# distributed-information-bottleneck/distributed-information-bottleneck.github.io

Hardware: NVIDIA H100
Metric: training samples/sec (16-feat synthetic, batch 65k) at 1/2/4/8 H100; HBM GB/s (higher is better)
Workload: dtype fp16 operands + fp32 accumulate (wgmma f16; PE/exp/KL/loss/Adam fp32)

## Files before the change

### distributed-information-bottleneck.github.io_b200/csrc/dib_enc_fused.cu

```cuda
#include <cuda.h>
#include <cuda_bf16.h>
#include <cuda_fp16.h>

#include "dib_common.cuh"
#include "dib_kernels.h"
#include "dib_sm90.cuh"

namespace {

using namespace sm90;

constexpr int TM = 128;
constexpr int HID = 128;
constexpr int EO = 64;
constexpr int K0 = 16;
constexpr int kThreads = 256;
constexpr int kPanel = TM * 128;

constexpr int kW0Elems = K0 * HID, kW1Elems = HID * HID, kW2Elems = HID * EO, kB1Elems = K0 * HID, kB2Elems = K0 * EO;
constexpr int kPackElems = kW0Elems + kW1Elems + kW2Elems + kB1Elems + kB2Elems;

constexpr int kOffW1 = 0;
constexpr int kOffW2 = kOffW1 + 2 * kPanel;
constexpr int kOffW0 = kOffW2 + kPanel;
constexpr int kOffBb1 = kOffW0 + 2 * K0 * 128;
constexpr int kOffBb2 = kOffBb1 + 2 * K0 * 128;
constexpr int kA0Bytes = 2 * TM * 16;
constexpr int kOffA0 = kOffBb2 + K0 * 128;
constexpr int kOffX = kOffA0 + 2 * kA0Bytes;
constexpr int kOffFwdEnd = kOffX + kThreads * 16;
constexpr int kOffH1 = kOffFwdEnd;
constexpr int kOffH2 = kOffH1 + 2 * kPanel;
constexpr int kOffDO = kOffH2 + 2 * kPanel;
constexpr int kOffDZ2 = kOffDO + kPanel;
constexpr int kOffG = kOffDZ2 + 2 * kPanel;
constexpr int kOffBwdEnd = kOffG + TM * 64;
static_assert(kOffH1 % 1024 == 0 && kOffDZ2 % 1024 == 0, "operand tiles must be 1024-byte aligned");

struct EncFusedParams {
  const float* x; int ldx;
  const int* x_off;
  const int* fdim;
  int nfreq;
  const float* params;
  const long long* b1_off; const long long* b2_off;
  const float* eps;
  unsigned long long seed; unsigned int step; unsigned long long sample_offset;
  const unsigned int* step_dev;
  float* emb; int ldemb; float* user_emb;
  uint16_t* emb16; int ldemb16;
  float* kl_part; int kl_stride;
  int F; long long n; int act; float alpha;
  int round_emb;
};

template <bool BF16>
__device__ __forceinline__ uint32_t pack2(float a, float b) {
  uint32_t r;
  if constexpr (BF16) asm("cvt.rn.satfinite.bf16x2.f32 %0, %1, %2;" : "=r"(r) : "f"(b), "f"(a));
  else asm("cvt.rn.satfinite.f16x2.f32 %0, %1, %2;" : "=r"(r) : "f"(b), "f"(a));
  return r;
}

template <bool BF16>
__device__ __forceinline__ uint32_t pack2_relu(float a, float b) {
  uint32_t r;
  if constexpr (BF16) asm("cvt.rn.relu.satfinite.bf16x2.f32 %0, %1, %2;" : "=r"(r) : "f"(b), "f"(a));
  else asm("cvt.rn.relu.satfinite.f16x2.f32 %0, %1, %2;" : "=r"(r) : "f"(b), "f"(a));
  return r;
}

template <bool BF16>
__device__ __forceinline__ void unpack2(uint32_t u, float& a, float& b) {
  if constexpr (BF16) { const float2 f = __bfloat1622float2(*reinterpret_cast<__nv_bfloat162*>(&u)); a = f.x; b = f.y; }
  else { const float2 f = __half22float2(*reinterpret_cast<__half2*>(&u)); a = f.x; b = f.y; }
}

__device__ __forceinline__ void st_shared_v4(uint32_t addr, uint32_t a, uint32_t b, uint32_t c, uint32_t d) {
  asm volatile("st.shared.v4.b32 [%0], {%1, %2, %3, %4};" ::"r"(addr), "r"(a), "r"(b), "r"(c), "r"(d) : "memory");
}
__device__ __forceinline__ void st_shared_b32(uint32_t addr, uint32_t v) {
  asm volatile("st.shared.b32 [%0], %1;" ::"r"(addr), "r"(v) : "memory");
}
__device__ __forceinline__ uint32_t ld_shared_b32(uint32_t addr) {
  uint32_t v;
  asm volatile("ld.shared.b32 %0, [%1];" : "=r"(v) : "r"(addr) : "memory");
  return v;
}

__device__ __forceinline__ uint32_t tile_chunk_addr(uint32_t tile, int r, int col) {
  const int panel = col >> 6, c = (col & 63) >> 3;
  return tile + panel * kPanel + r * 128 + ((c ^ (r & 7)) << 4);
}

struct Frag {
  int rb, q;
};
__device__ __forceinline__ Frag frag_of(int tid) {
  const int wg = tid >> 7, wq = (tid >> 5) & 3, lane = tid & 31;
  return Frag{64 * wg + 16 * wq + (lane >> 2), lane & 3};
}

template <bool BF16, bool RELU, int N>
__device__ __forceinline__ void frag_to_tile(const float (&d)[N / 2], uint32_t tile, Frag fr, int act, float alpha) {
#pragma unroll
  for (int j = 0; j < N / 8; ++j) {
#pragma unroll
    for (int h = 0; h < 2; ++h) {
      const float v0 = d[4 * j + 2 * h], v1 = d[4 * j + 2 * h + 1];
      const uint32_t w = RELU ? pack2_relu<BF16>(v0, v1) : pack2<BF16>(dib_act16(act, v0, alpha), dib_act16(act, v1, alpha));
      st_shared_b32(tile_chunk_addr(tile, fr.rb + 8 * h, 8 * j) + 4 * fr.q, w);
    }
  }
}

template <bool BF16, bool RELU, int N>
__device__ __forceinline__ void frag_to_a(const float (&d)[N / 2], uint32_t (&a)[N / 4], int act, float alpha) {
#pragma unroll
  for (int j = 0; j < N / 8; ++j) {
#pragma unroll
    for (int h = 0; h < 2; ++h) {
      const float v0 = d[4 * j + 2 * h], v1 = d[4 * j + 2 * h + 1];
      a[2 * j + h] = RELU ? pack2_relu<BF16>(v0, v1) : pack2<BF16>(dib_act16(act, v0, alpha), dib_act16(act, v1, alpha));
    }
  }
}

template <bool BF16>
__device__ __forceinline__ uint32_t relu_gate2(uint32_t p, uint32_t h) {
  if constexpr (BF16) {
    const __nv_bfloat162 z = __float2bfloat162_rn(0.f);
    __nv_bfloat162 g = __hmul2(*reinterpret_cast<__nv_bfloat162*>(&p), __hgt2(*reinterpret_cast<__nv_bfloat162*>(&h), z));
    return *reinterpret_cast<uint32_t*>(&g);
  } else {
    const __half2 z = __float2half2_rn(0.f);
    __half2 g = __hmul2(*reinterpret_cast<__half2*>(&p), __hgt2(*reinterpret_cast<__half2*>(&h), z));
    return *reinterpret_cast<uint32_t*>(&g);
  }
}

template <bool BF16, bool RELU>
__device__ __forceinline__ void frag_dgrad_to_tile(const float (&d)[64], uint32_t htile, uint32_t dtile, Frag fr, int act,
                                                   float alpha) {
#pragma unroll
  for (int j = 0; j < 16; ++j) {
#pragma unroll
    for (int h = 0; h < 2; ++h) {
      const uint32_t off = tile_chunk_addr(0u, fr.rb + 8 * h, 8 * j) + 4 * fr.q;
      const uint32_t hv = ld_shared_b32(htile + off);
      const float g0 = d[4 * j + 2 * h], g1 = d[4 * j + 2 * h + 1];
      uint32_t o;
      if constexpr (RELU) {
        o = relu_gate2<BF16>(pack2<BF16>(g0, g1), hv);
      } else {
        float h0, h1;
        unpack2<BF16>(hv, h0, h1);
        o = pack2<BF16>(g0 * dib_act_grad(act, h0, alpha), g1 * dib_act_grad(act, h1, alpha));
      }
      st_shared_b32(dtile + off, o);
    }
  }
}

__device__ __forceinline__ float dib_sin_pe(float a) {
  float t = a * 0.15915494309189535f;
  t -= rintf(t);
  return __sinf(6.283185307179586f * t);
}
constexpr int kMaxFeatDim = 3;
template <bool BF16>
__device__ __forceinline__ void write_a0_row(uint32_t a0, int r, int khalf, bool valid, const float (&xv)[kMaxFeatDim], int d,
                                             int nfreq) {
  float f[8];
  const int w_in = d * nfreq;
  int blk = (khalf * 8) / d, j = khalf * 8 - blk * d;
#pragma unroll
  for (int k = 0; k < 8; ++k) {
    const int col = khalf * 8 + k;
    float v = 0.f;
    if (col < w_in) {
      float xj = xv[0];
#pragma unroll
      for (int q = 1; q < kMaxFeatDim; ++q) if (j == q) xj = xv[q];
      v = blk == 0 ? xj : dib_sin_pe((float)(1 << blk) * xj);
    } else if (col == w_in) {
      v = valid ? 1.f : 0.f;
    }
    f[k] = v;
    if (++j == d) { j = 0; ++blk; }
  }
  st_shared_v4(a0 + khalf * (TM * 16) + r * 16, pack2<BF16>(f[0], f[1]), pack2<BF16>(f[2], f[3]), pack2<BF16>(f[4], f[5]),
               pack2<BF16>(f[6], f[7]));
}

__device__ __forceinline__ int a0_row(int tid) { return 64 * (tid >> 7) + (tid & 63); }

__device__ __forceinline__ void prefetch_x(const EncFusedParams& P, uint32_t xs, int tid, long long row0, int d, int xo) {
  const long long grow = row0 + a0_row(tid);
  if (grow < P.n) {
    const float* src = P.x + grow * P.ldx + xo;
#pragma unroll
    for (int j = 0; j < kMaxFeatDim; ++j)
      if (j < d) cp_async_4(xs + 4 * j, src + j);
  }
  cp_async_commit();
}
template <bool BF16>
__device__ __forceinline__ void stage_a0(const EncFusedParams& P, uint32_t a0, const float* xslot, int tid, long long row0,
                                         int d) {
  const int ar = a0_row(tid), khalf = (tid >> 6) & 1;
  const long long grow = row0 + ar;
  cp_async_wait_all();
  float xv[kMaxFeatDim];
#pragma unroll
  for (int j = 0; j < kMaxFeatDim; ++j) xv[j] = (grow < P.n && j < d) ? xslot[j] : 0.f;
  write_a0_row<BF16>(a0, ar, khalf, grow < P.n, xv, d, P.nfreq);
}

__device__ __forceinline__ void noise_pair(const EncFusedParams& P, unsigned int step, long long grow_lo, int f, int j, int q,
                                           int lane, float (&nz)[2][2]) {
  if (P.eps) {
#pragma unroll
    for (int h = 0; h < 2; ++h) {
      const long long grow = grow_lo + 8 * h;
      if (grow < P.n) {
        const float2 e = *reinterpret_cast<const float2*>(P.eps + (grow * P.F + f) * 32 + 8 * j + 2 * q);
        nz[h][0] = e.x; nz[h][1] = e.y;
      } else {
        nz[h][0] = nz[h][1] = 0.f;
      }
    }
    return;
  }
  float n4[4];
  dib_philox_normal4(P.seed, step, P.sample_offset + (unsigned long long)(grow_lo + 8 * (q & 1)), (uint32_t)f,
                     (uint32_t)(2 * j + (q >> 1)), n4);
#pragma unroll
  for (int h = 0; h < 2; ++h) {
    const int src = (lane & ~3) | ((q >> 1) << 1) | h;
    float t[4];
#pragma unroll
    for (int k = 0; k < 4; ++k) t[k] = __shfl_sync(0xffffffffu, n4[k], src);
    nz[h][0] = (q & 1) ? t[2] : t[0];
    nz[h][1] = (q & 1) ? t[3] : t[1];
  }
}

struct WeightMaps { CUtensorMap w0, w1, w2, b1, b2; };

__device__ __forceinline__ void load_weights(uint32_t sb, const WeightMaps& m, uint32_t bar, int f) {
  mbar_expect_tx(bar, 2 * K0 * 128 + 2 * kPanel + kPanel + 2 * K0 * 128 + K0 * 128);
  tma_load_3d(sb + kOffW0, &m.w0, bar, 0, 0, f);
  tma_load_3d(sb + kOffW0 + K0 * 128, &m.w0, bar, 64, 0, f);
  tma_load_3d(sb + kOffW1, &m.w1, bar, 0, 0, f);
  tma_load_3d(sb + kOffW1 + kPanel, &m.w1, bar, 64, 0, f);
  tma_load_3d(sb + kOffW2, &m.w2, bar, 0, 0, f);
  tma_load_3d(sb + kOffBb1, &m.b1, bar, 0, 0, f);
  tma_load_3d(sb + kOffBb1 + K0 * 128, &m.b1, bar, 64, 0, f);
  tma_load_3d(sb + kOffBb2, &m.b2, bar, 0, 0, f);
}

__device__ __forceinline__ uint64_t desc_a0_as_a(uint32_t a0, int wg) { return gmma_desc(a0 + wg * 64 * 16, TM * 16, 128, kLayoutNone); }
__device__ __forceinline__ uint64_t desc_a0_as_b(uint32_t a0, int kk) { return gmma_desc(a0 + kk * 256, 128, TM * 16, kLayoutNone); }
__device__ __forceinline__ uint64_t desc_act_as_a(uint32_t tile, int wg, int kk) {
  return gmma_desc(tile + (kk >> 2) * kPanel + wg * 64 * 128 + (kk & 3) * 32, 16, 1024);
}
__device__ __forceinline__ uint64_t desc_act_t_as_a(uint32_t tile, int p, int kk) { return gmma_desc(tile + p * kPanel + kk * 2048, kPanel, 1024); }
__device__ __forceinline__ uint64_t desc_act_as_b(uint32_t tile, int kk) { return gmma_desc(tile + kk * 2048, kPanel, 1024); }

template <bool BF16>
__device__ __forceinline__ void mma_layer0(float (&d)[64], uint32_t sb, uint32_t a0, int wg) {
  wgmma_m64n128k16<BF16, 0, 1>(d, desc_a0_as_a(a0, wg), gmma_desc(sb + kOffW0, K0 * 128, 1024), 0u);
}
template <bool BF16>
__device__ __forceinline__ void mma_layer1(float (&d)[64], uint32_t sb, uint32_t h1, uint32_t a0, int wg) {
  wgmma_m64n128k16<BF16, 0, 1>(d, desc_a0_as_a(a0, wg), gmma_desc(sb + kOffBb1, K0 * 128, 1024), 0u);
#pragma unroll
  for (int kk = 0; kk < HID / 16; ++kk)
    wgmma_m64n128k16<BF16, 0, 1>(d, desc_act_as_a(h1, wg, kk), gmma_desc(sb + kOffW1 + kk * 2048, kPanel, 1024), 1u);
}
template <bool BF16>
__device__ __forceinline__ void mma_layer2(float (&d)[32], uint32_t sb, uint32_t h2, uint32_t a0, int wg) {
  wgmma_m64n64k16<BF16, 0, 1>(d, desc_a0_as_a(a0, wg), gmma_desc(sb + kOffBb2, K0 * 128, 1024), 0u);
#pragma unroll
  for (int kk = 0; kk < HID / 16; ++kk)
    wgmma_m64n64k16<BF16, 0, 1>(d, desc_act_as_a(h2, wg, kk), gmma_desc(sb + kOffW2 + kk * 2048, kPanel, 1024), 1u);
}
template <bool BF16>
__device__ __forceinline__ void mma_layer1_rs(float (&d)[64], uint32_t sb, const uint32_t (&h1)[32], uint32_t a0, int wg) {
  wgmma_m64n128k16<BF16, 0, 1>(d, desc_a0_as_a(a0, wg), gmma_desc(sb + kOffBb1, K0 * 128, 1024), 0u);
#pragma unroll
  for (int kk = 0; kk < HID / 16; ++kk) {
    const uint32_t a[4] = {h1[4 * kk], h1[4 * kk + 1], h1[4 * kk + 2], h1[4 * kk + 3]};
    wgmma_m64n128k16_rs<BF16, 1>(d, a, gmma_desc(sb + kOffW1 + kk * 2048, kPanel, 1024), 1u);
  }
}
template <bool BF16>
__device__ __forceinline__ void mma_layer2_rs(float (&d)[32], uint32_t sb, const uint32_t (&h2)[32], uint32_t a0, int wg) {
  wgmma_m64n64k16<BF16, 0, 1>(d, desc_a0_as_a(a0, wg), gmma_desc(sb + kOffBb2, K0 * 128, 1024), 0u);
#pragma unroll
  for (int kk = 0; kk < HID / 16; ++kk) {
    const uint32_t a[4] = {h2[4 * kk], h2[4 * kk + 1], h2[4 * kk + 2], h2[4 * kk + 3]};
    wgmma_m64n64k16_rs<BF16, 1>(d, a, gmma_desc(sb + kOffW2 + kk * 2048, kPanel, 1024), 1u);
  }
}

__device__ __forceinline__ void wg_publish(int wg) {
  fence_proxy_async_smem();
  named_bar_sync(1 + wg, 128);
}
__device__ __forceinline__ void cta_publish() {
  fence_proxy_async_smem();
  __syncthreads();
}

struct Sched { int f_first, f_step, slot, nslots; };
__device__ __forceinline__ Sched sched_of(int c, int G, int F) {
  if (G >= F) { const int f0 = c % F; return Sched{f0, F * G, c / F, (G - f0 + F - 1) / F}; }
  return Sched{c, G, 0, 1};
}

template <bool BF16, bool RELU>
__global__ void __launch_bounds__(kThreads, 2)
dib_enc_fused_fwd_kernel(const __grid_constant__ WeightMaps maps, const EncFusedParams P) {
  extern __shared__ uint8_t smem_raw[];
  const uint32_t sb = (smem_u32(smem_raw) + 1023u) & ~1023u;
  uint8_t* sg = smem_raw + (sb - smem_u32(smem_raw));
  float* red_s = reinterpret_cast<float*>(sg + kOffFwdEnd + 64);
  const uint32_t bar_w = sb + kOffFwdEnd;

  const int tid = threadIdx.x, warp = tid >> 5, lane = tid & 31, wg = tid >> 7;
  const Frag fr = frag_of(tid);
  const int F = P.F;
  const int ntiles = (int)((P.n + TM - 1) / TM);
  const unsigned int nstep = P.step + (P.step_dev ? P.step_dev[0] : 0u);
  const uint32_t a0 = sb + kOffA0, xs = sb + kOffX + tid * 16;
  const float* xslot = reinterpret_cast<const float*>(sg + kOffX + tid * 16);

  if (tid == 0) {
    tma_prefetch_desc(&maps.w0); tma_prefetch_desc(&maps.w1); tma_prefetch_desc(&maps.w2);
    tma_prefetch_desc(&maps.b1); tma_prefetch_desc(&maps.b2);
    mbar_init(bar_w, 1);
    fence_barrier_init();
  }
  __syncthreads();

  const Sched s = sched_of(blockIdx.x, gridDim.x, F);
  uint32_t fit = 0;
  for (int f = s.f_first; f < F; f += s.f_step, ++fit) {
    if (tid == 0) load_weights(sb, maps, bar_w, f);
    const int d = P.fdim[f], xo = P.x_off[f];
    prefetch_x(P, xs, tid, (long long)s.slot * TM, d, xo);
    float kl_acc = 0.f;
    mbar_wait(bar_w, fit & 1);
    for (int t = s.slot; t < ntiles; t += s.nslots) {
      const long long row0 = (long long)t * TM;
      stage_a0<BF16>(P, a0, xslot, tid, row0, d);
      prefetch_x(P, xs, tid, row0 + (long long)s.nslots * TM, d, xo);
      wg_publish(wg);
      float acc[64];
      uint32_t ha[32];
      wgmma_fence();
      mma_layer0<BF16>(acc, sb, a0, wg);
      wgmma_commit();
      wgmma_wait<0>();
      wgmma_fence_regs(acc);
      frag_to_a<BF16, RELU, 128>(acc, ha, P.act, P.alpha);
      wgmma_fence();
      mma_layer1_rs<BF16>(acc, sb, ha, a0, wg);
      wgmma_commit();
      wgmma_wait<0>();
      wgmma_fence_regs(acc);
      frag_to_a<BF16, RELU, 128>(acc, ha, P.act, P.alpha);
      float acc2[32];
      wgmma_fence();
      mma_layer2_rs<BF16>(acc2, sb, ha, a0, wg);
      wgmma_commit();
      const long long grow_lo = row0 + fr.rb;
      float nz[4][2][2];
#pragma unroll
      for (int j = 0; j < 4; ++j) noise_pair(P, nstep, grow_lo, f, j, fr.q, lane, nz[j]);
      wgmma_wait<0>();
      wgmma_fence_regs(acc2);
#pragma unroll
      for (int h = 0; h < 2; ++h) {
        const long long grow = grow_lo + 8 * h;
        if (grow >= P.n) continue;
#pragma unroll
        for (int j = 0; j < 4; ++j) {
          const int e = 8 * j + 2 * fr.q;
          float u[2];
#pragma unroll
          for (int k = 0; k < 2; ++k) {
            const float mu = acc2[4 * j + 2 * h + k], lv = acc2[4 * (j + 4) + 2 * h + k];
            const float sv = __expf(0.5f * lv);
            u[k] = fmaf(sv, nz[j][h][k], mu);
            kl_acc += 0.5f * (mu * mu + sv * sv - lv - 1.f);
          }
          if (P.user_emb) *reinterpret_cast<float2*>(P.user_emb + grow * ((long long)F * 32) + f * 32 + e) = make_float2(u[0], u[1]);
          if (P.emb16) *reinterpret_cast<uint32_t*>(P.emb16 + grow * P.ldemb16 + f * 32 + e) = pack2<BF16>(u[0], u[1]);
          if (P.emb) {
            const float2 o = P.round_emb ? make_float2(dib_round_tf32(u[0]), dib_round_tf32(u[1])) : make_float2(u[0], u[1]);
            *reinterpret_cast<float2*>(P.emb + grow * P.ldemb + f * 32 + e) = o;
          }
        }
      }
    }
    kl_acc = dib_warp_sum(kl_acc);
    if (lane == 0) red_s[warp] = kl_acc;
    __syncthreads();
    if (tid == 0) {
      float sum = 0.f;
      for (int i = 0; i < kThreads / 32; ++i) sum += red_s[i];
      P.kl_part[(long long)f * P.kl_stride + s.slot] = sum;
    }
    __syncthreads();
  }
}

struct EncFusedBwdParams {
  EncFusedParams f;
  const float* d_emb; int ldd;
  const uint16_t* d_emb16;
  const float* beta_dev; float inv_batch; float gscale;
  float* part; long long split_stride;
  const long long* w0_off; const long long* b0_off; const long long* w1_off; const long long* w2_off;
};

__device__ __forceinline__ void load_demb16(uint32_t dst, const CUtensorMap* gmap, uint32_t bar, int f, long long row0) {
  mbar_expect_tx(bar, TM * 64);
  tma_load_2d(dst, gmap, bar, f * 32, (int)row0);
}

template <bool BF16, bool RELU>
__global__ void __launch_bounds__(kThreads, 1)
dib_enc_fused_bwd_kernel(const __grid_constant__ WeightMaps maps, const __grid_constant__ CUtensorMap gmap,
                         const EncFusedBwdParams Q) {
  const EncFusedParams& P = Q.f;
  extern __shared__ uint8_t smem_raw[];
  const uint32_t sb = (smem_u32(smem_raw) + 1023u) & ~1023u;
  const uint8_t* sg = smem_raw + (sb - smem_u32(smem_raw));
  const uint32_t bar_w = sb + kOffBwdEnd, bar_g = bar_w + 8;

  const int tid = threadIdx.x, lane = tid & 31, wg = tid >> 7;
  const Frag fr = frag_of(tid);
  const int F = P.F;
  const int ntiles = (int)((P.n + TM - 1) / TM);
  const unsigned int nstep = P.step + (P.step_dev ? P.step_dev[0] : 0u);
  const uint32_t h1 = sb + kOffH1, h2 = sb + kOffH2, dO = sb + kOffDO, dz2 = sb + kOffDZ2, gbuf = sb + kOffG;
  const uint32_t xs = sb + kOffX + tid * 16;
  const float* xslot = reinterpret_cast<const float*>(sg + kOffX + tid * 16);
  const uint32_t* gsm = reinterpret_cast<const uint32_t*>(sg + kOffG);
  const float S = Q.gscale, invS = 1.f / Q.gscale;

  if (tid == 0) {
    tma_prefetch_desc(&maps.w0); tma_prefetch_desc(&maps.w1); tma_prefetch_desc(&maps.w2);
    tma_prefetch_desc(&maps.b1); tma_prefetch_desc(&maps.b2);
    if (Q.d_emb16) tma_prefetch_desc(&gmap);
    mbar_init(bar_w, 1);
    mbar_init(bar_g, 1);
    fence_barrier_init();
  }
  __syncthreads();

  const Sched s = sched_of(blockIdx.x, gridDim.x, F);
  uint32_t fit = 0, tpar = 0;
  for (int f = s.f_first; f < F; f += s.f_step, ++fit) {
    if (tid == 0) {
      load_weights(sb, maps, bar_w, f);
      if (Q.d_emb16 && s.slot < ntiles) load_demb16(gbuf, &gmap, bar_g, f, (long long)s.slot * TM);
    }
    const int d = P.fdim[f], xo = P.x_off[f];
    prefetch_x(P, xs, tid, (long long)s.slot * TM, d, xo);
    const float bs = Q.beta_dev[0] * Q.inv_batch * S;
    float accW1[64], accW2[32], accW0[8], accB1[8], accB2[8];
    mbar_wait(bar_w, fit & 1);
    for (int t = s.slot; t < ntiles; t += s.nslots) {
      const long long row0 = (long long)t * TM;
      const uint32_t wacc = t != s.slot;
      const uint32_t a0 = sb + kOffA0 + tpar * kA0Bytes;
      stage_a0<BF16>(P, a0, xslot, tid, row0, d);
      prefetch_x(P, xs, tid, row0 + (long long)s.nslots * TM, d, xo);
      wg_publish(wg);
      float acc[64];
      wgmma_fence();
      mma_layer0<BF16>(acc, sb, a0, wg);
      wgmma_commit();
      wgmma_wait<0>();
      wgmma_fence_regs(acc); wgmma_fence_regs(accW0);
      frag_to_tile<BF16, RELU, 128>(acc, h1, fr, P.act, P.alpha);
      cta_publish();
      wgmma_fence();
      mma_layer1<BF16>(acc, sb, h1, a0, wg);
      wgmma_commit();
      wgmma_wait<0>();
      wgmma_fence_regs(acc);
      frag_to_tile<BF16, RELU, 128>(acc, h2, fr, P.act, P.alpha);
      wg_publish(wg);
      float acc2[32];
      wgmma_fence();
      mma_layer2<BF16>(acc2, sb, h2, a0, wg);
      wgmma_commit();
      const long long grow_lo = row0 + fr.rb;
      float nz[4][2][2];
#pragma unroll
      for (int j = 0; j < 4; ++j) noise_pair(P, nstep, grow_lo, f, j, fr.q, lane, nz[j]);
      if (Q.d_emb16) mbar_wait(bar_g, tpar);
      wgmma_wait<0>();
      wgmma_fence_regs(acc2);
#pragma unroll
      for (int h = 0; h < 2; ++h) {
        const long long grow = grow_lo + 8 * h;
        const bool valid = grow < P.n;
        const float bsv = valid ? bs : 0.f;
        const int r = fr.rb + 8 * h;
#pragma unroll
        for (int j = 0; j < 4; ++j) {
          const int e = 8 * j + 2 * fr.q;
          float g[2] = {0.f, 0.f};
          if (valid) {
            if (Q.d_emb16) unpack2<BF16>(gsm[r * 16 + e / 2], g[0], g[1]);
            else {
              const float2 g2 = *reinterpret_cast<const float2*>(Q.d_emb + grow * Q.ldd + f * 32 + e);
              g[0] = g2.x * S; g[1] = g2.y * S;
            }
          }
          float dm[2], dl[2];
#pragma unroll
          for (int k = 0; k < 2; ++k) {
            const float mu = acc2[4 * j + 2 * h + k], lv = acc2[4 * (j + 4) + 2 * h + k];
            const float sgm = expf(0.5f * lv);
            dm[k] = fmaf(bsv, mu, g[k]);
            dl[k] = valid ? fmaf(g[k] * nz[j][h][k], 0.5f * sgm, bsv * 0.5f * (sgm * sgm - 1.f)) : 0.f;
          }
          st_shared_b32(tile_chunk_addr(dO, r, e) + 4 * fr.q, pack2<BF16>(dm[0], dm[1]));
          st_shared_b32(tile_chunk_addr(dO, r, 32 + e) + 4 * fr.q, pack2<BF16>(dl[0], dl[1]));
        }
      }
      cta_publish();
      if (tid == 0 && Q.d_emb16 && t + s.nslots < ntiles) load_demb16(gbuf, &gmap, bar_g, f, row0 + (long long)s.nslots * TM);
      wgmma_fence();
#pragma unroll
      for (int kk = 0; kk < EO / 16; ++kk)
        wgmma_m64n128k16<BF16, 0, 0>(acc, gmma_desc(dO + wg * 64 * 128 + kk * 32, 16, 1024),
                                     gmma_desc(sb + kOffW2 + kk * 32, 16, 1024), kk > 0 ? 1u : 0u);
      wgmma_commit();
#pragma unroll
      for (int kk = 0; kk < TM / 16; ++kk)
        wgmma_m64n64k16<BF16, 1, 1>(accW2, desc_act_t_as_a(h2, wg, kk), desc_act_as_b(dO, kk), kk > 0 ? 1u : wacc);
#pragma unroll
      for (int kk = 0; kk < TM / 16; ++kk)
        wgmma_m64n16k16<BF16, 1, 1>(accB2, desc_act_t_as_a(dO, 0, kk), desc_a0_as_b(a0, kk), kk > 0 ? 1u : wacc);
      wgmma_commit();
      wgmma_wait<1>();
      wgmma_fence_regs(acc);
      frag_dgrad_to_tile<BF16, RELU>(acc, h2, dz2, fr, P.act, P.alpha);
      wgmma_wait<0>();
      wgmma_fence_regs(accW2); wgmma_fence_regs(accB2);
      cta_publish();
      wgmma_fence();
#pragma unroll
      for (int kk = 0; kk < HID / 16; ++kk)
        wgmma_m64n128k16<BF16, 0, 0>(acc, desc_act_as_a(dz2, wg, kk),
                                     gmma_desc(sb + kOffW1 + (kk >> 2) * kPanel + (kk & 3) * 32, 16, 1024), kk > 0 ? 1u : 0u);
      wgmma_commit();
#pragma unroll
      for (int kk = 0; kk < TM / 16; ++kk)
        wgmma_m64n128k16<BF16, 1, 1>(accW1, desc_act_t_as_a(h1, wg, kk), desc_act_as_b(dz2, kk), kk > 0 ? 1u : wacc);
#pragma unroll
      for (int kk = 0; kk < TM / 16; ++kk)
        wgmma_m64n16k16<BF16, 1, 1>(accB1, desc_act_t_as_a(dz2, wg, kk), desc_a0_as_b(a0, kk), kk > 0 ? 1u : wacc);
      wgmma_commit();
      wgmma_wait<1>();
      wgmma_fence_regs(acc);
      frag_dgrad_to_tile<BF16, RELU>(acc, h1, h2, fr, P.act, P.alpha);
      wgmma_wait<0>();
      wgmma_fence_regs(accW1); wgmma_fence_regs(accB1);
      cta_publish();
      wgmma_fence();
#pragma unroll
      for (int kk = 0; kk < TM / 16; ++kk)
        wgmma_m64n16k16<BF16, 1, 1>(accW0, desc_act_t_as_a(h2, wg, kk), desc_a0_as_b(a0, kk), kk > 0 ? 1u : wacc);
      wgmma_commit();
      tpar ^= 1u;
    }
    wgmma_wait<0>();
    wgmma_fence_regs(accW0);
    float* part = Q.part + (long long)s.slot * Q.split_stride;
    const int w_in = d * P.nfreq;
    const bool ran = s.slot < ntiles;
    auto out = [&](float v) { return ran ? v * invS : 0.f; };
#pragma unroll
    for (int h = 0; h < 2; ++h) {
      const int m = fr.rb + 8 * h;
#pragma unroll
      for (int j = 0; j < 16; ++j)
        *reinterpret_cast<float2*>(part + Q.w1_off[f] + (long long)m * HID + 8 * j + 2 * fr.q) =
            make_float2(out(accW1[4 * j + 2 * h]), out(accW1[4 * j + 2 * h + 1]));
#pragma unroll
      for (int j = 0; j < 8; ++j)
        *reinterpret_cast<float2*>(part + Q.w2_off[f] + (long long)m * EO + 8 * j + 2 * fr.q) =
            make_float2(out(accW2[4 * j + 2 * h]), out(accW2[4 * j + 2 * h + 1]));
#pragma unroll
      for (int j = 0; j < 2; ++j) {
#pragma unroll
        for (int k = 0; k < 2; ++k) {
          const int col = 8 * j + 2 * fr.q + k;
          const float v0 = out(accW0[4 * j + 2 * h + k]);
          if (col < w_in) part[Q.w0_off[f] + (long long)col * HID + m] = v0;
          else if (col == w_in) {
            part[Q.b0_off[f] + m] = v0;
            part[P.b1_off[f] + m] = out(accB1[4 * j + 2 * h + k]);
            if (wg == 0) part[P.b2_off[f] + m] = out(accB2[4 * j + 2 * h + k]);
          }
        }
      }
    }
    __syncthreads();
  }
}

template <bool BF16>
__global__ void dib_enc_pack_weights_kernel(const float* __restrict__ params, const long long* __restrict__ w0_off,
                                            const long long* __restrict__ b0_off, const long long* __restrict__ w1_off,
                                            const long long* __restrict__ b1_off, const long long* __restrict__ w2_off,
                                            const long long* __restrict__ b2_off, const int* __restrict__ fdim, int nfreq,
                                            float logvar_offset, uint16_t* __restrict__ out, float* __restrict__ zero, long long zero_n) {
  const int f = blockIdx.y;
  int i = blockIdx.x * blockDim.x + threadIdx.x;
  {
    const long long z = ((long long)f * gridDim.x + blockIdx.x) * blockDim.x + threadIdx.x;
    if (z < zero_n) zero[z] = 0.f;
  }
  if (i >= kPackElems) return;
  const int idx = i, w_in = fdim[f] * nfreq;
  float v;
  if (i < kW0Elems) {
    const int k = i / HID, n = i - k * HID;
    v = k < w_in ? params[w0_off[f] + (long long)k * HID + n] : (k == w_in ? params[b0_off[f] + n] : 0.f);
  } else if ((i -= kW0Elems) < kW1Elems) {
    v = params[w1_off[f] + i];
  } else if ((i -= kW1Elems) < kW2Elems) {
    v = params[w2_off[f] + i];
  } else if ((i -= kW2Elems) < kB1Elems) {
    const int k = i / HID, n = i - k * HID;
    v = k == w_in ? params[b1_off[f] + n] : 0.f;
  } else {
    i -= kB1Elems;
    const int k = i / EO, n = i - k * EO;
    v = k == w_in ? params[b2_off[f] + n] + (n >= EO / 2 ? logvar_offset : 0.f) : 0.f;
  }
  out[(long long)f * kPackElems + idx] = (uint16_t)(pack2<BF16>(v, 0.f) & 0xffffu);
}

typedef CUresult (*EncodeTiledFn)(CUtensorMap*, CUtensorMapDataType, cuuint32_t, void*, const cuuint64_t*,
                                  const cuuint64_t*, const cuuint32_t*, const cuuint32_t*, CUtensorMapInterleave,
                                  CUtensorMapSwizzle, CUtensorMapL2promotion, CUtensorMapFloatOOBfill);
EncodeTiledFn encode_fn2() {
  static EncodeTiledFn fn = nullptr;
  if (!fn) {
    void* p = nullptr;
    cudaDriverEntryPointQueryResult q;
    if (cudaGetDriverEntryPoint("cuTensorMapEncodeTiled", &p, cudaEnableDefault, &q) == cudaSuccess &&
        q == cudaDriverEntryPointSuccess)
      fn = reinterpret_cast<EncodeTiledFn>(p);
// ... 106 lines not shown
```

### distributed-information-bottleneck.github.io_b200/csrc/dib_sm90.cuh

```cuda
#pragma once
#include <cuda_runtime.h>
#include <stdint.h>

namespace sm90 {

__device__ __forceinline__ uint32_t smem_u32(const void* p) { return (uint32_t)__cvta_generic_to_shared(p); }

__device__ __forceinline__ void mbar_init(uint32_t bar, uint32_t count) {
  asm volatile("mbarrier.init.shared::cta.b64 [%0], %1;" ::"r"(bar), "r"(count) : "memory");
}
__device__ __forceinline__ void fence_barrier_init() {
  asm volatile("fence.mbarrier_init.release.cluster;" ::: "memory");
}
__device__ __forceinline__ void mbar_expect_tx(uint32_t bar, uint32_t bytes) {
  asm volatile("mbarrier.arrive.expect_tx.shared::cta.b64 _, [%0], %1;" ::"r"(bar), "r"(bytes) : "memory");
}
__device__ __forceinline__ void mbar_arrive(uint32_t bar) {
  asm volatile("mbarrier.arrive.shared::cta.b64 _, [%0];" ::"r"(bar) : "memory");
}
__device__ __forceinline__ bool mbar_try_wait(uint32_t bar, uint32_t parity) {
  uint32_t ok;
  asm volatile(
      "{\n\t.reg .pred p;\n\t"
      "mbarrier.try_wait.parity.shared::cta.b64 p, [%1], %2;\n\t"
      "selp.u32 %0, 1, 0, p;\n\t}"
      : "=r"(ok) : "r"(bar), "r"(parity) : "memory");
  return ok != 0;
}
__device__ __forceinline__ void mbar_wait(uint32_t bar, uint32_t parity) {
  while (!mbar_try_wait(bar, parity)) {}
}

__device__ __forceinline__ void named_bar_sync(uint32_t id, uint32_t count) {
  asm volatile("bar.sync %0, %1;" ::"r"(id), "r"(count) : "memory");
}

__device__ __forceinline__ void tma_prefetch_desc(const void* map) {
  asm volatile("prefetch.tensormap [%0];" ::"l"(map) : "memory");
}
__device__ __forceinline__ void tma_load_2d(uint32_t dst, const void* map, uint32_t bar, int c0, int c1) {
  asm volatile(
      "cp.async.bulk.tensor.2d.shared::cluster.global.tile.mbarrier::complete_tx::bytes [%0], [%1, {%3, %4}], [%2];"
      ::"r"(dst), "l"(map), "r"(bar), "r"(c0), "r"(c1) : "memory");
}
__device__ __forceinline__ void tma_load_3d(uint32_t dst, const void* map, uint32_t bar, int c0, int c1, int c2) {
  asm volatile(
      "cp.async.bulk.tensor.3d.shared::cluster.global.tile.mbarrier::complete_tx::bytes [%0], [%1, {%3, %4, %5}], [%2];"
      ::"r"(dst), "l"(map), "r"(bar), "r"(c0), "r"(c1), "r"(c2) : "memory");
}
__device__ __forceinline__ void tma_store_2d(const void* map, uint32_t src, int c0, int c1) {
  asm volatile("cp.async.bulk.tensor.2d.global.shared::cta.bulk_group [%0, {%2, %3}], [%1];"
               ::"l"(map), "r"(src), "r"(c0), "r"(c1) : "memory");
}
__device__ __forceinline__ void bulk_commit() { asm volatile("cp.async.bulk.commit_group;" ::: "memory"); }
template <int N>
__device__ __forceinline__ void bulk_wait_read() { asm volatile("cp.async.bulk.wait_group.read %0;" ::"n"(N) : "memory"); }
__device__ __forceinline__ void bulk_wait_all() { asm volatile("cp.async.bulk.wait_group 0;" ::: "memory"); }
__device__ __forceinline__ void cp_async_4(uint32_t dst, const void* src) {
  asm volatile("cp.async.ca.shared.global [%0], [%1], 4;" ::"r"(dst), "l"(src) : "memory");
}
__device__ __forceinline__ void cp_async_commit() { asm volatile("cp.async.commit_group;" ::: "memory"); }
__device__ __forceinline__ void cp_async_wait_all() { asm volatile("cp.async.wait_group 0;" ::: "memory"); }

__device__ __forceinline__ void fence_proxy_async_smem() {
  asm volatile("fence.proxy.async.shared::cta;" ::: "memory");
}

__device__ __forceinline__ void wgmma_fence() { asm volatile("wgmma.fence.sync.aligned;" ::: "memory"); }
__device__ __forceinline__ void wgmma_commit() { asm volatile("wgmma.commit_group.sync.aligned;" ::: "memory"); }
template <int N>
__device__ __forceinline__ void wgmma_wait() { asm volatile("wgmma.wait_group.sync.aligned %0;" ::"n"(N) : "memory"); }
template <int N>
__device__ __forceinline__ void wgmma_fence_regs(float (&d)[N]) {
#pragma unroll
  for (int i = 0; i < N; ++i) asm volatile("" : "+f"(d[i])::"memory");
}

constexpr uint32_t kLayoutSw128 = 1, kLayoutNone = 0;
__device__ __forceinline__ uint64_t gmma_desc(uint32_t smem_addr, uint32_t lbo_bytes, uint32_t sbo_bytes,
                                              uint32_t layout_type = kLayoutSw128) {
  uint64_t d = 0;
  d |= (uint64_t)((smem_addr & 0x3FFFF) >> 4);
  d |= (uint64_t)((lbo_bytes >> 4) & 0x3FFF) << 16;
  d |= (uint64_t)((sbo_bytes >> 4) & 0x3FFF) << 32;
  d |= (uint64_t)layout_type << 62;
  return d;
}

template <bool BF16, int TA, int TB>
__device__ __forceinline__ void wgmma_m64n16k16(float (&d)[8], uint64_t da, uint64_t db, uint32_t accumulate) {
  if constexpr (BF16) {
    asm volatile(
        "{\n\t.reg .pred p;\n\tsetp.ne.b32 p, %10, 0;\n\t"
        "wgmma.mma_async.sync.aligned.m64n16k16.f32.bf16.bf16 {%0, %1, %2, %3, %4, %5, %6, %7}, %8, %9, p, 1, 1, %11, %12;\n\t}"
        : "+f"(d[0]), "+f"(d[1]), "+f"(d[2]), "+f"(d[3]), "+f"(d[4]), "+f"(d[5]), "+f"(d[6]), "+f"(d[7])
        : "l"(da), "l"(db), "r"(accumulate), "n"(TA), "n"(TB)
        : "memory");
  } else {
    asm volatile(
        "{\n\t.reg .pred p;\n\tsetp.ne.b32 p, %10, 0;\n\t"
        "wgmma.mma_async.sync.aligned.m64n16k16.f32.f16.f16 {%0, %1, %2, %3, %4, %5, %6, %7}, %8, %9, p, 1, 1, %11, %12;\n\t}"
        : "+f"(d[0]), "+f"(d[1]), "+f"(d[2]), "+f"(d[3]), "+f"(d[4]), "+f"(d[5]), "+f"(d[6]), "+f"(d[7])
        : "l"(da), "l"(db), "r"(accumulate), "n"(TA), "n"(TB)
        : "memory");
  }
}

template <bool BF16, int TA, int TB>
__device__ __forceinline__ void wgmma_m64n64k16(float (&d)[32], uint64_t da, uint64_t db, uint32_t accumulate) {
  if constexpr (BF16) {
    asm volatile(
        "{\n\t.reg .pred p;\n\tsetp.ne.b32 p, %34, 0;\n\t"
        "wgmma.mma_async.sync.aligned.m64n64k16.f32.bf16.bf16 {%0, %1, %2, %3, %4, %5, %6, %7, %8, %9, %10, %11, %12, %13, %14, %15, %16, %17, %18, %19, %20, %21, %22, %23, %24, %25, %26, %27, %28, %29, %30, %31}, %32, %33, p, 1, 1, %35, %36;\n\t}"
        : "+f"(d[0]), "+f"(d[1]), "+f"(d[2]), "+f"(d[3]), "+f"(d[4]), "+f"(d[5]), "+f"(d[6]), "+f"(d[7]), "+f"(d[8]), "+f"(d[9]), "+f"(d[10]), "+f"(d[11]), "+f"(d[12]), "+f"(d[13]), "+f"(d[14]), "+f"(d[15]), "+f"(d[16]), "+f"(d[17]), "+f"(d[18]), "+f"(d[19]), "+f"(d[20]), "+f"(d[21]), "+f"(d[22]), "+f"(d[23]), "+f"(d[24]), "+f"(d[25]), "+f"(d[26]), "+f"(d[27]), "+f"(d[28]), "+f"(d[29]), "+f"(d[30]), "+f"(d[31])
        : "l"(da), "l"(db), "r"(accumulate), "n"(TA), "n"(TB)
        : "memory");
  } else {
// ... 105 lines not shown
```

Baseline: 60.90 million.

## Replace CTA-wide syncs with split arrive/wait barriers and register-sourced wgmma

Swaps the __syncthreads-based publishes between the two warpgroups for paired named-barrier arrive/wait events, so each warpgroup only waits for its peer's tile right before reading it. Activations and gradients are kept in register fragments and fed to register-sourced (RS) wgmma for the forward layers and the output dgrad, with the shared tiles still written for the transposed weight-gradient GEMMs. Tile addressing is precomputed per thread, with an opaque helper that stops the compiler re-deriving it. This aims to cut barrier stalls and shared-memory round trips, but adds register pressure and more intricate barrier ordering that could hide races.

```diff
diff --git a/distributed-information-bottleneck.github.io_b200/csrc/dib_enc_fused.cu b/distributed-information-bottleneck.github.io_b200/csrc/dib_enc_fused.cu
--- a/distributed-information-bottleneck.github.io_b200/csrc/dib_enc_fused.cu
+++ b/distributed-information-bottleneck.github.io_b200/csrc/dib_enc_fused.cu
@@ -88,11 +88,6 @@
   return v;
 }
 
-__device__ __forceinline__ uint32_t tile_chunk_addr(uint32_t tile, int r, int col) {
-  const int panel = col >> 6, c = (col & 63) >> 3;
-  return tile + panel * kPanel + r * 128 + ((c ^ (r & 7)) << 4);
-}
-
 struct Frag {
   int rb, q;
 };
@@ -101,17 +96,19 @@
   return Frag{64 * wg + 16 * wq + (lane >> 2), lane & 3};
 }
 
-template <bool BF16, bool RELU, int N>
-__device__ __forceinline__ void frag_to_tile(const float (&d)[N / 2], uint32_t tile, Frag fr, int act, float alpha) {
-#pragma unroll
-  for (int j = 0; j < N / 8; ++j) {
-#pragma unroll
-    for (int h = 0; h < 2; ++h) {
-      const float v0 = d[4 * j + 2 * h], v1 = d[4 * j + 2 * h + 1];
-      const uint32_t w = RELU ? pack2_relu<BF16>(v0, v1) : pack2<BF16>(dib_act16(act, v0, alpha), dib_act16(act, v1, alpha));
-      st_shared_b32(tile_chunk_addr(tile, fr.rb + 8 * h, 8 * j) + 4 * fr.q, w);
-    }
-  }
+__device__ __forceinline__ uint32_t opaque(uint32_t v) {
+  asm volatile("" : "+r"(v));
+  return v;
+}
+
+struct FragWords {
+  uint32_t base, sw;
+};
+__device__ __forceinline__ FragWords frag_words(uint32_t tile, Frag fr) {
+  return FragWords{opaque(tile + fr.rb * 128 + 4 * fr.q), opaque((fr.rb & 7) << 4)};
+}
+__device__ __forceinline__ uint32_t frag_word_addr(FragWords fw, int j, int h) {
+  return fw.base + (j >> 3) * kPanel + h * 1024 + (((j & 7) << 4) ^ fw.sw);
 }
 
 template <bool BF16, bool RELU, int N>
@@ -123,6 +120,16 @@
       const float v0 = d[4 * j + 2 * h], v1 = d[4 * j + 2 * h + 1];
       a[2 * j + h] = RELU ? pack2_relu<BF16>(v0, v1) : pack2<BF16>(dib_act16(act, v0, alpha), dib_act16(act, v1, alpha));
     }
+  }
+}
+
+template <int N>
+__device__ __forceinline__ void a_to_tile(const uint32_t (&a)[N / 4], uint32_t tile, Frag fr) {
+  const FragWords fw = frag_words(tile, fr);
+#pragma unroll
+  for (int j = 0; j < N / 8; ++j) {
+#pragma unroll
+    for (int h = 0; h < 2; ++h) st_shared_b32(frag_word_addr(fw, j, h), a[2 * j + h]);
   }
 }
 
@@ -140,24 +147,22 @@
 }
 
 template <bool BF16, bool RELU>
-__device__ __forceinline__ void frag_dgrad_to_tile(const float (&d)[64], uint32_t htile, uint32_t dtile, Frag fr, int act,
-                                                   float alpha) {
+__device__ __forceinline__ void frag_dgrad_to_a(const float (&d)[64], uint32_t htile, uint32_t (&a)[32], Frag fr, int act,
+                                                float alpha) {
+  const FragWords fw = frag_words(htile, fr);
 #pragma unroll
   for (int j = 0; j < 16; ++j) {
 #pragma unroll
     for (int h = 0; h < 2; ++h) {
-      const uint32_t off = tile_chunk_addr(0u, fr.rb + 8 * h, 8 * j) + 4 * fr.q;
-      const uint32_t hv = ld_shared_b32(htile + off);
+      const uint32_t hv = ld_shared_b32(frag_word_addr(fw, j, h));
       const float g0 = d[4 * j + 2 * h], g1 = d[4 * j + 2 * h + 1];
-      uint32_t o;
       if constexpr (RELU) {
-        o = relu_gate2<BF16>(pack2<BF16>(g0, g1), hv);
+        a[2 * j + h] = relu_gate2<BF16>(pack2<BF16>(g0, g1), hv);
       } else {
         float h0, h1;
         unpack2<BF16>(hv, h0, h1);
-        o = pack2<BF16>(g0 * dib_act_grad(act, h0, alpha), g1 * dib_act_grad(act, h1, alpha));
-      }
-      st_shared_b32(dtile + off, o);
+        a[2 * j + h] = pack2<BF16>(g0 * dib_act_grad(act, h0, alpha), g1 * dib_act_grad(act, h1, alpha));
+      }
     }
   }
 }
@@ -273,20 +278,6 @@
   wgmma_m64n128k16<BF16, 0, 1>(d, desc_a0_as_a(a0, wg), gmma_desc(sb + kOffW0, K0 * 128, 1024), 0u);
 }
 template <bool BF16>
-__device__ __forceinline__ void mma_layer1(float (&d)[64], uint32_t sb, uint32_t h1, uint32_t a0, int wg) {
-  wgmma_m64n128k16<BF16, 0, 1>(d, desc_a0_as_a(a0, wg), gmma_desc(sb + kOffBb1, K0 * 128, 1024), 0u);
-#pragma unroll
-  for (int kk = 0; kk < HID / 16; ++kk)
-    wgmma_m64n128k16<BF16, 0, 1>(d, desc_act_as_a(h1, wg, kk), gmma_desc(sb + kOffW1 + kk * 2048, kPanel, 1024), 1u);
-}
-template <bool BF16>
-__device__ __forceinline__ void mma_layer2(float (&d)[32], uint32_t sb, uint32_t h2, uint32_t a0, int wg) {
-  wgmma_m64n64k16<BF16, 0, 1>(d, desc_a0_as_a(a0, wg), gmma_desc(sb + kOffBb2, K0 * 128, 1024), 0u);
-#pragma unroll
-  for (int kk = 0; kk < HID / 16; ++kk)
-    wgmma_m64n64k16<BF16, 0, 1>(d, desc_act_as_a(h2, wg, kk), gmma_desc(sb + kOffW2 + kk * 2048, kPanel, 1024), 1u);
-}
-template <bool BF16>
 __device__ __forceinline__ void mma_layer1_rs(float (&d)[64], uint32_t sb, const uint32_t (&h1)[32], uint32_t a0, int wg) {
   wgmma_m64n128k16<BF16, 0, 1>(d, desc_a0_as_a(a0, wg), gmma_desc(sb + kOffBb1, K0 * 128, 1024), 0u);
 #pragma unroll
@@ -309,10 +300,12 @@
   fence_proxy_async_smem();
   named_bar_sync(1 + wg, 128);
 }
-__device__ __forceinline__ void cta_publish() {
+constexpr uint32_t kEvL0 = 3, kEvDO = 5, kEvDZ2 = 7, kEvDW2 = 9, kEvDZ1 = 11;
+__device__ __forceinline__ void xwg_arrive(uint32_t e, int wg) {
   fence_proxy_async_smem();
-  __syncthreads();
-}
+  named_bar_arrive(e + wg, 256);
+}
+__device__ __forceinline__ void xwg_wait(uint32_t e, int wg) { named_bar_sync(e + (wg ^ 1), 256); }
 
 struct Sched { int f_first, f_step, slot, nslots; };
 __device__ __forceinline__ Sched sched_of(int c, int G, int F) {
@@ -450,7 +443,6 @@
   const uint32_t h1 = sb + kOffH1, h2 = sb + kOffH2, dO = sb + kOffDO, dz2 = sb + kOffDZ2, gbuf = sb + kOffG;
   const uint32_t xs = sb + kOffX + tid * 16;
   const float* xslot = reinterpret_cast<const float*>(sg + kOffX + tid * 16);
-  const uint32_t* gsm = reinterpret_cast<const uint32_t*>(sg + kOffG);
   const float S = Q.gscale, invS = 1.f / Q.gscale;
 
   if (tid == 0) {
@@ -488,18 +480,22 @@
       wgmma_commit();
       wgmma_wait<0>();
       wgmma_fence_regs(acc); wgmma_fence_regs(accW0);
-      frag_to_tile<BF16, RELU, 128>(acc, h1, fr, P.act, P.alpha);
-      cta_publish();
+      xwg_arrive(kEvL0, wg);
+      uint32_t ha[32];
+      frag_to_a<BF16, RELU, 128>(acc, ha, P.act, P.alpha);
+      a_to_tile<128>(ha, h1, fr);
+      float acc1[64];
       wgmma_fence();
-      mma_layer1<BF16>(acc, sb, h1, a0, wg);
+      mma_layer1_rs<BF16>(acc1, sb, ha, a0, wg);
       wgmma_commit();
       wgmma_wait<0>();
-      wgmma_fence_regs(acc);
-      frag_to_tile<BF16, RELU, 128>(acc, h2, fr, P.act, P.alpha);
-      wg_publish(wg);
+      wgmma_fence_regs(acc1);
+      frag_to_a<BF16, RELU, 128>(acc1, ha, P.act, P.alpha);
+      xwg_wait(kEvL0, wg);
+      a_to_tile<128>(ha, h2, fr);
       float acc2[32];
       wgmma_fence();
-      mma_layer2<BF16>(acc2, sb, h2, a0, wg);
+      mma_layer2_rs<BF16>(acc2, sb, ha, a0, wg);
       wgmma_commit();
       const long long grow_lo = row0 + fr.rb;
       float nz[4][2][2];
@@ -508,6 +504,7 @@
       if (Q.d_emb16) mbar_wait(bar_g, tpar);
       wgmma_wait<0>();
       wgmma_fence_regs(acc2);
+      uint32_t ao[16];
 #pragma unroll
       for (int h = 0; h < 2; ++h) {
         const long long grow = grow_lo + 8 * h;
@@ -519,7 +516,7 @@
           const int e = 8 * j + 2 * fr.q;
           float g[2] = {0.f, 0.f};
           if (valid) {
-            if (Q.d_emb16) unpack2<BF16>(gsm[r * 16 + e / 2], g[0], g[1]);
+            if (Q.d_emb16) unpack2<BF16>(ld_shared_b32(gbuf + 4 * (r * 16 + e / 2)), g[0], g[1]);
             else {
               const float2 g2 = *reinterpret_cast<const float2*>(Q.d_emb + grow * Q.ldd + f * 32 + e);
               g[0] = g2.x * S; g[1] = g2.y * S;
@@ -533,54 +530,79 @@
             dm[k] = fmaf(bsv, mu, g[k]);
             dl[k] = valid ? fmaf(g[k] * nz[j][h][k], 0.5f * sgm, bsv * 0.5f * (sgm * sgm - 1.f)) : 0.f;
           }
-          st_shared_b32(tile_chunk_addr(dO, r, e) + 4 * fr.q, pack2<BF16>(dm[0], dm[1]));
-          st_shared_b32(tile_chunk_addr(dO, r, 32 + e) + 4 * fr.q, pack2<BF16>(dl[0], dl[1]));
+          ao[2 * j + h] = pack2<BF16>(dm[0], dm[1]);
+          ao[8 + 2 * j + h] = pack2<BF16>(dl[0], dl[1]);
         }
       }
-      cta_publish();
+      a_to_tile<64>(ao, dO, fr);
+      xwg_arrive(kEvDO, wg);
+      float accd[64];
+      wgmma_fence();
+#pragma unroll
+      for (int kk = 0; kk < EO / 16; ++kk) {
+        const uint32_t a[4] = {ao[4 * kk], ao[4 * kk + 1], ao[4 * kk + 2], ao[4 * kk + 3]};
+        wgmma_m64n128k16_rs<BF16, 0>(accd, a, gmma_desc(sb + kOffW2 + kk * 32, 16, 1024), kk > 0 ? 1u : 0u);
+      }
+      wgmma_commit();
+      xwg_wait(kEvDO, wg);
       if (tid == 0 && Q.d_emb16 && t + s.nslots < ntiles) load_demb16(gbuf, &gmap, bar_g, f, row0 + (long long)s.nslots * TM);
+      {
+        const uint32_t h2o = opaque(h2), dOo = opaque(dO), a0o = opaque(a0);
+        wgmma_fence();
+#pragma unroll
+        for (int kk = 0; kk < TM / 16; ++kk)
+          wgmma_m64n64k16<BF16, 1, 1>(accW2, desc_act_t_as_a(h2o, wg, kk), desc_act_as_b(dOo, kk), kk > 0 ? 1u : wacc);
+#pragma unroll
+        for (int kk = 0; kk < TM / 16; ++kk)
+          wgmma_m64n16k16<BF16, 1, 1>(accB2, desc_act_t_as_a(dOo, 0, kk), desc_a0_as_b(a0o, kk), kk > 0 ? 1u : wacc);
+      }
+      wgmma_commit();
+      wgmma_wait<1>();
+      wgmma_fence_regs(accd);
+      {
+        uint32_t az[32];
+        frag_dgrad_to_a<BF16, RELU>(accd, h2, az, fr, P.act, P.alpha);
+        a_to_tile<128>(az, dz2, fr);
+      }
+      xwg_arrive(kEvDZ2, wg);
+      float accg[64];
+      wg_publish(wg);
       wgmma_fence();
 #pragma unroll
-      for (int kk = 0; kk < EO / 16; ++kk)
-        wgmma_m64n128k16<BF16, 0, 0>(acc, gmma_desc(dO + wg * 64 * 128 + kk * 32, 16, 1024),
-                                     gmma_desc(sb + kOffW2 + kk * 32, 16, 1024), kk > 0 ? 1u : 0u);
-      wgmma_commit();
-#pragma unroll
-      for (int kk = 0; kk < TM / 16; ++kk)
-        wgmma_m64n64k16<BF16, 1, 1>(accW2, desc_act_t_as_a(h2, wg, kk), desc_act_as_b(dO, kk), kk > 0 ? 1u : wacc);
-#pragma unroll
-      for (int kk = 0; kk < TM / 16; ++kk)
-        wgmma_m64n16k16<BF16, 1, 1>(accB2, desc_act_t_as_a(dO, 0, kk), desc_a0_as_b(a0, kk), kk > 0 ? 1u : wacc);
+      for (int kk = 0; kk < HID / 16; ++kk)
+        wgmma_m64n128k16<BF16, 0, 0>(accg, desc_act_as_a(dz2, wg, kk),
+                                     gmma_desc(sb + kOffW1 + (kk >> 2) * kPanel + (kk & 3) * 32, 16, 1024), kk > 0 ? 1u : 0u);
+      wgmma_commit();
+      xwg_wait(kEvDZ2, wg);
+      {
+        const uint32_t h1o = opaque(h1), dz2o = opaque(dz2), a0o = opaque(a0);
+        wgmma_fence();
+#pragma unroll
+        for (int kk = 0; kk < TM / 16; ++kk)
+          wgmma_m64n128k16<BF16, 1, 1>(accW1, desc_act_t_as_a(h1o, wg, kk), desc_act_as_b(dz2o, kk), kk > 0 ? 1u : wacc);
+#pragma unroll
+        for (int kk = 0; kk < TM / 16; ++kk)
+          wgmma_m64n16k16<BF16, 1, 1>(accB1, desc_act_t_as_a(dz2o, wg, kk), desc_a0_as_b(a0o, kk), kk > 0 ? 1u : wacc);
+      }
       wgmma_commit();
       wgmma_wait<1>();
-      wgmma_fence_regs(acc);
-      frag_dgrad_to_tile<BF16, RELU>(acc, h2, dz2, fr, P.act, P.alpha);
-      wgmma_wait<0>();
-      wgmma_fence_regs(accW2); wgmma_fence_regs(accB2);
-      cta_publish();
-      wgmma_fence();
-#pragma unroll
-      for (int kk = 0; kk < HID / 16; ++kk)
-        wgmma_m64n128k16<BF16, 0, 0>(acc, desc_act_as_a(dz2, wg, kk),
-                                     gmma_desc(sb + kOffW1 + (kk >> 2) * kPanel + (kk & 3) * 32, 16, 1024), kk > 0 ? 1u : 0u);
-      wgmma_commit();
-#pragma unroll
-      for (int kk = 0; kk < TM / 16; ++kk)
-        wgmma_m64n128k16<BF16, 1, 1>(accW1, desc_act_t_as_a(h1, wg, kk), desc_act_as_b(dz2, kk), kk > 0 ? 1u : wacc);
-#pragma unroll
-      for (int kk = 0; kk < TM / 16; ++kk)
-        wgmma_m64n16k16<BF16, 1, 1>(accB1, desc_act_t_as_a(dz2, wg, kk), desc_a0_as_b(a0, kk), kk > 0 ? 1u : wacc);
-      wgmma_commit();
-      wgmma_wait<1>();
-      wgmma_fence_regs(acc);
-      frag_dgrad_to_tile<BF16, RELU>(acc, h1, h2, fr, P.act, P.alpha);
+      wgmma_fence_regs(accg); wgmma_fence_regs(accW2); wgmma_fence_regs(accB2);
+      xwg_arrive(kEvDW2, wg);
+      uint32_t az[32];
+      frag_dgrad_to_a<BF16, RELU>(accg, h1, az, fr, P.act, P.alpha);
+      xwg_wait(kEvDW2, wg);
+      a_to_tile<128>(az, h2, fr);
       wgmma_wait<0>();
       wgmma_fence_regs(accW1); wgmma_fence_regs(accB1);
-      cta_publish();
-      wgmma_fence();
-#pragma unroll
-      for (int kk = 0; kk < TM / 16; ++kk)
-        wgmma_m64n16k16<BF16, 1, 1>(accW0, desc_act_t_as_a(h2, wg, kk), desc_a0_as_b(a0, kk), kk > 0 ? 1u : wacc);
+      xwg_arrive(kEvDZ1, wg);
+      xwg_wait(kEvDZ1, wg);
+      {
+        const uint32_t h2o = opaque(h2), a0o = opaque(a0);
+        wgmma_fence();
+#pragma unroll
+        for (int kk = 0; kk < TM / 16; ++kk)
+          wgmma_m64n16k16<BF16, 1, 1>(accW0, desc_act_t_as_a(h2o, wg, kk), desc_a0_as_b(a0o, kk), kk > 0 ? 1u : wacc);
+      }
       wgmma_commit();
       tpar ^= 1u;
     }
diff --git a/distributed-information-bottleneck.github.io_b200/csrc/dib_sm90.cuh b/distributed-information-bottleneck.github.io_b200/csrc/dib_sm90.cuh
--- a/distributed-information-bottleneck.github.io_b200/csrc/dib_sm90.cuh
+++ b/distributed-information-bottleneck.github.io_b200/csrc/dib_sm90.cuh
@@ -33,6 +33,9 @@
 
 __device__ __forceinline__ void named_bar_sync(uint32_t id, uint32_t count) {
   asm volatile("bar.sync %0, %1;" ::"r"(id), "r"(count) : "memory");
+}
+__device__ __forceinline__ void named_bar_arrive(uint32_t id, uint32_t count) {
+  asm volatile("bar.arrive %0, %1;" ::"r"(id), "r"(count) : "memory");
 }
 
 __device__ __forceinline__ void tma_prefetch_desc(const void* map) {
```

New measurement: 65.33 million, median of 6. 7.3% higher.
